# pawanjay176/kzg_rust

Measured on AMD Instinct MI355X. Metric: blobs/sec on verify_blob_kzg_proof_batch (mainnet 4096, batch=64), higher is better.
Workload: dtype u32 limbs (29-bit) / 64-bit accumulate, u8 bytes

## Files before the change

### __graft_entry__.py

```python
import os
import subprocess
import sys

ROOT = os.path.dirname(os.path.abspath(__file__))
if ROOT not in sys.path:
    sys.path.insert(0, ROOT)


def build() -> None:
    env = dict(os.environ)
    subprocess.run(["make", "-C", os.path.join(ROOT, "kzg_rust_amd", "csrc"), "-j5"], check=True, env=env)
    subprocess.run(["make", "-C", os.path.join(ROOT, "oracle")], check=True, env=env)
    native = os.path.join(ROOT, "tests", "native")
    subprocess.run(["g++", "-O2", "-shared", "-fPIC", "-o", os.path.join(native, "libhd_probe.so"), os.path.join(native, "hd_probe.cpp")],
                   check=True, env=env)
    subprocess.run(["g++", "-O2", "-shared", "-fPIC", "-o", os.path.join(native, "liblazy_chain_probe.so"), os.path.join(native, "lazy_chain_probe.cpp")],
                   check=True, env=env)
    subprocess.run(["g++", "-std=c++17", "-O2", "-o", os.path.join(native, "cpp_vector_runner"), os.path.join(native, "cpp_vector_runner.cpp"),
                    "-L" + os.path.join(ROOT, "kzg_rust_amd"), "-lkzg355", "-Wl,-rpath," + os.path.join(ROOT, "kzg_rust_amd")], check=True, env=env)
    subprocess.run(["g++", "-std=c++17", "-O2", "-o", os.path.join(native, "cpp_cell_runner"), os.path.join(native, "cpp_cell_runner.cpp"),
                    "-L" + os.path.join(ROOT, "kzg_rust_amd"), "-lkzg355", "-Wl,-rpath," + os.path.join(ROOT, "kzg_rust_amd")], check=True, env=env)
    subprocess.run(["g++", "-std=c++17", "-O2", "-o", os.path.join(native, "cpp_cell_compute_runner"), os.path.join(native, "cpp_cell_compute_runner.cpp"),
                    "-L" + os.path.join(ROOT, "kzg_rust_amd"), "-lkzg355", "-Wl,-rpath," + os.path.join(ROOT, "kzg_rust_amd")], check=True, env=env)
    subprocess.run(["g++", "-std=c++17", "-O2", "-o", os.path.join(native, "cpp_cell_recover_runner"), os.path.join(native, "cpp_cell_recover_runner.cpp"),
                    "-L" + os.path.join(ROOT, "kzg_rust_amd"), "-lkzg355", "-Wl,-rpath," + os.path.join(ROOT, "kzg_rust_amd")], check=True, env=env)
    quad_src, quad_bin = os.path.join(native, "quad_ops_test.hip"), os.path.join(native, "quad_ops_test")
    quad_deps = [quad_src] + [os.path.join(ROOT, "kzg_rust_amd", "csrc", f) for f in ("g1_quad.h", "g1.h", "field.h", "modinv.h", "consts_gen.h")]
    if not os.path.exists(quad_bin) or any(os.path.getmtime(d) > os.path.getmtime(quad_bin) for d in quad_deps):
        subprocess.run(["/opt/rocm/bin/hipcc", "-O3", "-std=c++17", "--offload-arch=gfx950", "-Wno-unused-result", "-o", quad_bin, quad_src], check=True, env=env)
    probe_src, probe_so = os.path.join(native, "gpu_probe.hip"), os.path.join(native, "libgpu_probe.so")
    probe_deps = [probe_src] + [os.path.join(ROOT, "kzg_rust_amd", "csrc", f) for f in ("field.h", "modinv.h", "eval_core.h", "consts_gen.h")]
    if not os.path.exists(probe_so) or any(os.path.getmtime(d) > os.path.getmtime(probe_so) for d in probe_deps):
        subprocess.run(["/opt/rocm/bin/hipcc", "-O3", "-std=c++17", "--offload-arch=gfx950", "-Wno-unused-result", "-shared", "-fPIC", "-o", probe_so, probe_src],
                       check=True, env=env)
    group_src, group_so = os.path.join(native, "gpu_group_probe.hip"), os.path.join(native, "libgpu_group_probe.so")
    group_deps = [group_src] + [os.path.join(ROOT, "kzg_rust_amd", "csrc", f) for f in
                                ("field.h", "modinv.h", "tower.h", "g1.h", "pairing.h", "pairing_coop.h", "pairing_lanes.h", "consts_gen.h")]
    if not os.path.exists(group_so) or any(os.path.getmtime(d) > os.path.getmtime(group_so) for d in group_deps):
        subprocess.run(["/opt/rocm/bin/hipcc", "-O3", "-std=c++17", "--offload-arch=gfx950", "-Wno-unused-result", "-shared", "-fPIC", "-o", group_so, group_src],
                       check=True, env=env)
    import kzg_rust_amd
    from kzg_rust_amd import _lib
    lib = _lib.load()
    for name in _lib.EXPORTED_SYMBOLS:
        getattr(lib, name)
    print("build ok:", lib.kzg355_version().decode())


def smoke() -> None:
    import torch
    assert torch.cuda.is_available(), "smoke() needs a GPU"
    import kzg_rust_amd as kz
    from oracle.oracle import Oracle
    sys.path.insert(0, os.path.join(ROOT, "tests"))
    from synth import random_blob
    golden = os.path.join(ROOT, "tests", "golden")
    g1 = open(os.path.join(golden, "trusted_setup_g1.bin"), "rb").read()
    g2 = open(os.path.join(golden, "trusted_setup_g2.bin"), "rb").read()
    s = kz.Kzg.load_trusted_setup([g1[48 * i:48 * i + 48] for i in range(4096)], [g2[96 * i:96 * i + 96] for i in range(65)])
    o = Oracle()
    os_ = o.load_trusted_setup(g1, g2)
    blobs = [random_blob(1000 + i) for i in range(3)]
    cs = [kz.Kzg.blob_to_kzg_commitment(kz.Blob(b), s) for b in blobs]
    assert [c.to_bytes() for c in cs] == [o.blob_to_kzg_commitment(b, os_) for b in blobs], "commitment mismatch vs oracle"
    ps = [kz.Kzg.compute_blob_kzg_proof(kz.Blob(b), c, s) for b, c in zip(blobs, cs)]
    assert [p.to_bytes() for p in ps] == [o.compute_blob_kzg_proof(b, c.to_bytes(), os_) for b, c in zip(blobs, cs)], "proof mismatch vs oracle"
    ok = kz.Kzg.verify_blob_kzg_proof_batch([kz.Blob(b) for b in blobs], cs, ps, s)
    assert ok is True and o.verify_blob_kzg_proof_batch(blobs, [c.to_bytes() for c in cs], [p.to_bytes() for p in ps], os_) is True
    bad = [ps[1], ps[0], ps[2]]
    assert kz.Kzg.verify_blob_kzg_proof_batch([kz.Blob(b) for b in blobs], cs, bad, s) is False
    s.free()
    o.free_trusted_setup(os_)
    print("smoke ok: commit/prove bit-exact vs oracle, verify batch true/false as expected")


if __name__ == "__main__":
    build()
    if len(sys.argv) > 1 and sys.argv[1] == "smoke":
        smoke()
```

### kzg_rust_amd/csrc/g1.h

```cpp
#pragma once
#include "field.h"

#if defined(KZG_MID_INLINE)
#define KZG_G1_MID KZG_HD
#else
#define KZG_G1_MID KZG_HD_NOINLINE
#endif

namespace kzg {

struct G1Affine { Fp x, y; };
struct G1Jac { Fp x, y, z; };

KZG_HD G1Jac g1_inf() { G1Jac r; r.x = fp_zero(); r.y = fp_zero(); r.z = fp_zero(); return r; }
KZG_HD G1Affine g1a_inf() { G1Affine r; r.x = fp_zero(); r.y = fp_zero(); return r; }
KZG_HD bool g1_is_inf(const G1Jac &a) { return fp_is_zero(a.z); }
KZG_HD bool g1a_is_inf(const G1Affine &a) { return fp_is_zero(a.x) && fp_is_zero(a.y); }
KZG_HD void g1_neg(G1Jac &r, const G1Jac &a) { r.x = a.x; r.z = a.z; fp_neg(r.y, a.y); }
KZG_HD void g1a_neg(G1Affine &r, const G1Affine &a) { r.x = a.x; fp_neg(r.y, a.y); }
KZG_HD void g1_from_affine(G1Jac &r, const G1Affine &a) {
    bool inf = g1a_is_inf(a);
    r.x = a.x; r.y = a.y;
    Fp one = fp_one(), zero = fp_zero();
    fp_select(r.z, inf, one, zero);
// ... 34 lines not shown
    fp_sub(H, U2, a.x);
    fp_sub(R, S2, a.y);
    if (fp_is_zero(H)) {
        if (fp_is_zero(R)) { G1Jac d = a; g1_dbl(r, d); } else { r = g1_inf(); }
        return;
    }
    fp_sqr(HH, H); fp_mul(HHH, H, HH); fp_mul(V, a.x, HH);
    Fp X3, Y3;
    fp_sqr(X3, R); fp_sub(X3, X3, HHH); fp_sub(X3, X3, V); fp_sub(X3, X3, V);
    fp_sub(t, V, X3); fp_mul(Y3, R, t);
    fp_mul(t, a.y, HHH); fp_sub(Y3, Y3, t);
    fp_mul(r.z, a.z, H);
    r.x = X3; r.y = Y3;
}

KZG_G1_MID void g1_add(G1Jac &r, const G1Jac &a, const G1Jac &b) {
    if (g1_is_inf(a)) { r = b; return; }
    if (g1_is_inf(b)) { r = a; return; }
    Fp Z1Z1, Z2Z2, U1, U2, S1, S2, H, R, HH, HHH, V, t;
    fp_sqr(Z1Z1, a.z); fp_sqr(Z2Z2, b.z);
    fp_mul(U1, a.x, Z2Z2); fp_mul(U2, b.x, Z1Z1);
    fp_mul(S1, a.y, b.z); fp_mul(S1, S1, Z2Z2);
    fp_mul(S2, b.y, a.z); fp_mul(S2, S2, Z1Z1);
    fp_sub(H, U2, U1);
    fp_sub(R, S2, S1);
    if (fp_is_zero(H)) {
        if (fp_is_zero(R)) { G1Jac d = a; g1_dbl(r, d); } else { r = g1_inf(); }
        return;
    }
    fp_sqr(HH, H); fp_mul(HHH, H, HH); fp_mul(V, U1, HH);
    Fp X3, Y3, Z3;
    fp_sqr(X3, R); fp_sub(X3, X3, HHH); fp_sub(X3, X3, V); fp_sub(X3, X3, V);
    fp_sub(t, V, X3); fp_mul(Y3, R, t);
    fp_mul(t, S1, HHH); fp_sub(Y3, Y3, t);
    fp_mul(Z3, a.z, b.z); fp_mul(Z3, Z3, H);
    r.x = X3; r.y = Y3; r.z = Z3;
}

struct G1X { Fp x, y, zz, zzz; };
KZG_HD G1X g1x_inf() { G1X r; r.x = fp_zero(); r.y = fp_zero(); r.zz = fp_zero(); r.zzz = fp_zero(); return r; }
KZG_HD bool g1x_is_inf(const G1X &a) { return fp_is_zero(a.zz); }
KZG_G1_MID void g1x_add_mixed(G1X &r, const G1X &a, const G1Affine &b) {
    if (g1a_is_inf(b)) { r = a; return; }
    if (g1x_is_inf(a)) { r.x = b.x; r.y = b.y; r.zz = fp_one(); r.zzz = fp_one(); return; }
    Fp U2, S2, P, R, PP, PPP, Q, t;
    fp_mul(U2, b.x, a.zz);
    fp_mul(S2, b.y, a.zzz);
    fp_sub(P, U2, a.x);
    fp_sub(R, S2, a.y);
    if (fp_is_zero(P)) {
        if (!fp_is_zero(R)) { r = g1x_inf(); return; }
        Fp U, V, W, S, M;
        fp_dbl(U, b.y); fp_sqr(V, U); fp_mul(W, U, V); fp_mul(S, b.x, V);
        fp_sqr(M, b.x); fp_dbl(t, M); fp_add(M, M, t);
        Fp X3, Y3;
        fp_sqr(X3, M); fp_sub(X3, X3, S); fp_sub(X3, X3, S);
        fp_sub(t, S, X3); fp_mul(Y3, M, t); fp_mul(t, W, b.y); fp_sub(Y3, Y3, t);
        r.x = X3; r.y = Y3; r.zz = V; r.zzz = W;
        return;
    }
    fp_sqr(PP, P); fp_mul(PPP, P, PP); fp_mul(Q, a.x, PP);
    Fp X3, Y3;
    fp_sqr(X3, R); fp_sub(X3, X3, PPP); fp_sub(X3, X3, Q); fp_sub(X3, X3, Q);
    fp_sub(t, Q, X3); fp_mul(Y3, R, t);
    fp_mul(t, a.y, PPP); fp_sub(Y3, Y3, t);
    fp_mul(r.zz, a.zz, PP);
    fp_mul(r.zzz, a.zzz, PPP);
    r.x = X3; r.y = Y3;
}
KZG_HD void g1_lazy_x3(Fp &X3, Fp &t, const Fp &RR, const Fp &PPP, const Fp &Q) {
    const uint32_t m2[NFP] = FP_MOD2_INIT, m8[NFP] = FP_MOD8_INIT;
    Fp u;
    fp_sub_lz(t, RR, PPP, m2);
    fp_sub_lz(u, t, Q, m2);
    fp_sub_lz(X3, u, Q, m2);
    fp_sub_lz(t, Q, X3, m8);
}
KZG_HD void g1_lazy_y3(Fp &Y3, const Fp &R, const Fp &t, const Fp &S1, const Fp &PPP) {
    const uint32_t m2[NFP] = FP_MOD2_INIT;
    Fp u;
    { const Fp z = fp_zero(); fp_sub_lz(u, z, S1, m2); }
    fp_mul2_lz(Y3, R, t, u, PPP);
}
KZG_G1_MID void g1x_add_mixed_lazy(G1X &acc, bool &started, const G1Affine &b) {
    const uint32_t m2[NFP] = FP_MOD2_INIT, m4[NFP] = FP_MOD4_INIT, m8[NFP] = FP_MOD8_INIT;
    if (!started) {
        if (g1a_is_inf(b)) return;
        acc.x = b.x; acc.y = b.y; acc.zz = fp_one(); acc.zzz = fp_one(); started = true;
        return;
    }
    Fp U2, S2, P, R;
    fp_mul_lz(U2, b.x, acc.zz);
    fp_mul_lz(S2, b.y, acc.zzz);
    fp_sub_lz(P, U2, acc.x, m8);
    fp_sub_lz(R, S2, acc.y, m4);
    if (fp_maybe_zero_lz(P) || g1a_is_inf(b)) {
        G1X c; fp_canon16(c.x, acc.x); fp_canon16(c.y, acc.y); fp_canon16(c.zz, acc.zz); fp_canon16(c.zzz, acc.zzz);
        g1x_add_mixed(c, c, b);
        acc = c;
        started = !g1x_is_inf(c);
        return;
    }
    Fp PP, PPP, Q, t, u;
    fp_sqr_lz(PP, P); fp_mul_lz(PPP, P, PP); fp_mul_lz(Q, acc.x, PP);
    Fp X3, Y3;
    fp_sqr_lz(X3, R);
    fp_sub_lz(t, X3, PPP, m2);
    fp_sub_lz(u, t, Q, m2);
    fp_sub_lz(X3, u, Q, m2);
    fp_sub_lz(t, Q, X3, m8);
#if defined(KZG_G1_ADD_MUL2)
    { const Fp z = fp_zero(); fp_sub_lz(u, z, acc.y, m4); }
    fp_mul2_lz(Y3, R, t, u, PPP);
#else
    fp_mul_lz(Y3, R, t);
    fp_mul_lz(t, acc.y, PPP);
    fp_sub_lz(Y3, Y3, t, m2);
#endif
    fp_mul_lz(acc.zz, acc.zz, PP);
    fp_mul_lz(acc.zzz, acc.zzz, PPP);
    acc.x = X3; acc.y = Y3;
}
KZG_G1_MID void g1x_from_lazy(G1X &r, const G1X &acc, bool started) {
    if (!started) { r = g1x_inf(); return; }
    fp_canon16(r.x, acc.x); fp_canon16(r.y, acc.y); fp_canon16(r.zz, acc.zz); fp_canon16(r.zzz, acc.zzz);
}

KZG_G1_MID void g1x_to_jac(G1Jac &r, const G1X &a) {
    if (g1x_is_inf(a)) { r = g1_inf(); return; }
    fp_mul(r.x, a.x, a.zz);
    fp_mul(r.y, a.y, a.zzz);
    r.z = a.zz;
}

KZG_G1_MID void g1x_add_lazy2(G1X &r, const G1X &a, const G1X &b) {
    const uint32_t m2[NFP] = FP_MOD2_INIT;
    Fp U1, U2, S1, S2, ZZ12, ZZZ12, P, R;
    fp_mul_lz(U1, a.x, b.zz); fp_mul_lz(U2, b.x, a.zz);
    fp_mul_lz(S1, a.y, b.zzz); fp_mul_lz(S2, b.y, a.zzz);
    fp_mul_lz(ZZ12, a.zz, b.zz); fp_mul_lz(ZZZ12, a.zzz, b.zzz);
    fp_sub_lz(P, U2, U1, m2);
    fp_sub_lz(R, S2, S1, m2);
    if (fp_maybe_zero_lz(P) || fp_maybe_zero_lz(a.zz) || fp_maybe_zero_lz(b.zz)) {
        G1X ca, cb; g1x_from_lazy(ca, a, true); g1x_from_lazy(cb, b, true);
        G1Jac ja, jb, jr; g1x_to_jac(ja, ca); g1x_to_jac(jb, cb);
        g1_add(jr, ja, jb);
        if (g1_is_inf(jr)) { r = g1x_inf(); return; }
        r.x = jr.x; r.y = jr.y; fp_sqr(r.zz, jr.z); fp_mul(r.zzz, r.zz, jr.z);
        return;
    }
    Fp PP, PPP, Q, t, X3, Y3;
    fp_sqr_lz(PP, P); fp_mul_lz(PPP, P, PP); fp_mul_lz(Q, U1, PP);
    fp_sqr_lz(X3, R);
    g1_lazy_x3(X3, t, X3, PPP, Q);
    g1_lazy_y3(Y3, R, t, S1, PPP);
    fp_mul_lz(r.zz, ZZ12, PP);
    fp_mul_lz(r.zzz, ZZZ12, PPP);
    r.x = X3; r.y = Y3;
}


struct PairPt { Fp ax, ay, az; };
KZG_G1_MID void pairpt_from_jac(PairPt &r, const G1Jac &a, bool negate) {
    if (g1_is_inf(a)) { r.ax = fp_zero(); r.ay = fp_zero(); r.az = fp_zero(); return; }
    Fp z2;
    fp_mul(r.ax, a.x, a.z);
    fp_sqr(z2, a.z); fp_mul(r.az, z2, a.z);
    r.ay = a.y;
    if (negate) fp_neg(r.ay, r.ay);
}
KZG_HD void pairpt_from_affine(PairPt &r, const G1Affine &a) {
    if (g1a_is_inf(a)) { r.ax = fp_zero(); r.ay = fp_zero(); r.az = fp_zero(); return; }
    r.ax = a.x; r.ay = a.y; r.az = fp_one();
}
KZG_G1_MID void g1_to_affine(G1Affine &r, const G1Jac &a) {
    if (g1_is_inf(a)) { r = g1a_inf(); return; }
    Fp zi, zi2, zi3;
    fp_inv(zi, a.z); fp_sqr(zi2, zi); fp_mul(zi3, zi2, zi);
    fp_mul(r.x, a.x, zi2); fp_mul(r.y, a.y, zi3);
}
KZG_G1_MID void pairpt_to_affine(G1Affine &r, const PairPt &a) {
    if (fp_is_zero(a.az)) { r = g1a_inf(); return; }
    Fp zi; fp_inv(zi, a.az);
    fp_mul(r.x, a.ax, zi); fp_mul(r.y, a.ay, zi);
}

KZG_HD void g1_mul_words(G1Jac &r, const G1Affine &p, const uint32_t *k, int nwords) {
    G1Jac acc = g1_inf();
    for (int w = nwords - 1; w >= 0; w--) {
        uint32_t x = k[w];
        for (int b = 0; b < 32; b++) {
            g1_dbl(acc, acc);
            if (x >> 31) g1_add_mixed(acc, acc, p);
            x <<= 1;
        }
    }
    r = acc;
}

KZG_G1_MID void g1_dbl_lazy(G1Jac &r, const G1Jac &p) {
    const uint32_t m2[NFP] = FP_MOD2_INIT, m4[NFP] = FP_MOD4_INIT, m8[NFP] = FP_MOD8_INIT;
// ... 239 lines not shown
```

### kzg_rust_amd/csrc/k_g1.hip

```cpp
#if !defined(KZG_G1_TU_NOINLINE)
#define KZG_MID_INLINE 1
#else
#define KZG_FP_MUL_NOINLINE 1
#endif
#include "kernels.h"
#include "g1_quad.h"

namespace kzg {

template <bool SUBGROUP>
__device__ __forceinline__ void decode_point_to_slot(const uint8_t *commitments, const uint8_t *proofs, int n_total, int n_per_group, G1Affine *pts, int *err,
        int stride) {
    const int j = blockIdx.x * blockDim.x + threadIdx.x;
    if (j >= 2 * n_total) return;
    const bool is_proof = j >= n_total;
    if (is_proof && !proofs) return;
    const int i = is_proof ? j - n_total : j;
    const uint8_t *src = (is_proof ? proofs : commitments) + (size_t)stride * i;
    uint8_t b[48];
    for (int k = 0; k < 48; k++) b[k] = src[k];
    G1Affine p;
    int rc = g1_decompress(p, b);
    if (SUBGROUP && rc == 0 && !g1a_is_inf(p) && !g1_in_subgroup(p)) rc = 3;
    const int g = i / n_per_group, k = i % n_per_group;
// ... 127 lines not shown
    if (c >= 2) return;
    G1Jac acc = g1_inf();
    for (int wv = 0; wv < wpg; wv++) { G1Jac v = partials[((size_t)g * wpg + wv) * 2 + c]; g1_add(acc, acc, v); }
    PairPt a; pairpt_from_jac(a, acc, c == 0);
    pair_pts[2 * (size_t)g + c] = a;
}

__global__ void __launch_bounds__(64) k_lincomb_single(const G1Affine *pts, const uint32_t *scal_b, const uint32_t *scal_c, int groups, PairPt *pair_pts,
                                                        uint32_t *wtabs) {
    const int lane = threadIdx.x, q = lane & 3;
    const int g_raw = blockIdx.x * 16 + (lane >> 2);
    const bool live = g_raw < groups;
    const int g = live ? g_raw : groups - 1;
    uint32_t *wtab = wtabs + (size_t)blockIdx.x * (W4_ENTRIES * 3 * NFP * 64);
    const G1Affine *gp = pts + 2 * (size_t)g;
    G1Affine p; uint32_t k[8];
    if (q < 2) { p = gp[1]; for (int w = 0; w < 8; w++) k[w] = scal_b[8 * (size_t)g + w]; }
    else { p = g1a_neg_gen(); for (int w = 0; w < 8; w++) k[w] = scal_c[8 * (size_t)g + w]; }
    uint32_t ka[4], kb[4];
    glv_split_fast(ka, kb, k);
    if (q & 1) { G1Affine t; g1a_neg_phi(t, p); p = t; }
    G1Jac m;
    g1_mul128_w4(m, p, (q & 1) ? kb : ka, wtab, lane);
    G1Jac c; g1_from_affine(c, gp[0]);
#pragma unroll 1
    for (int it = 0; it < 3; it++) {
        G1Jac o = g1_shfl_xor(m, it == 0 ? 1 : 2);
        if (it == 2) o = c;
        g1_add(m, m, o);
    }
    if (!live) return;
    if (q == 0) { PairPt a; pairpt_from_jac(a, m, false); pair_pts[2 * (size_t)g + 1] = a; }
    if (q == 1) {
        G1Jac pj; g1_from_affine(pj, gp[1]);
        PairPt a; pairpt_from_jac(a, pj, true); pair_pts[2 * (size_t)g] = a;
    }
}

constexpr int LC_BITS = 5;
constexpr int LC_BUCKETS = 1 << (LC_BITS - 1);
constexpr int LC_WINDOWS = 26;
constexpr int LC_DIG_STRIDE = 28;
__host__ __device__ inline int lc_items(int n) { return 2 * (3 * n + 1); }

__global__ void __launch_bounds__(64) k_lc_prep(const G1Affine *pts, const uint32_t *scal_a, const uint32_t *scal_b, const uint32_t *scal_c, int n,
                                                 G1Affine *items, int8_t *digits) {
    const int nt = 3 * n + 1, bpg = (nt + 63) / 64;
    const int g = blockIdx.x / bpg, t = (blockIdx.x % bpg) * 64 + threadIdx.x;
    if (t >= nt) return;
    const G1Affine *gp = pts + (size_t)g * 2 * n;
    G1Affine p; uint32_t k[8];
    if (t < n) { p = gp[n + t]; for (int q = 0; q < 8; q++) k[q] = scal_a[8 * ((size_t)g * n + t) + q]; }
    else if (t < 2 * n) { p = gp[n + (t - n)]; for (int q = 0; q < 8; q++) k[q] = scal_b[8 * ((size_t)g * n + (t - n)) + q]; }
    else if (t < 3 * n) { p = gp[t - 2 * n]; for (int q = 0; q < 8; q++) k[q] = scal_a[8 * ((size_t)g * n + (t - 2 * n)) + q]; }
    else { p = g1a_neg_gen(); for (int q = 0; q < 8; q++) k[q] = scal_c[8 * (size_t)g + q]; }
    uint32_t half[2][4];
    glv_split(half[0], half[1], k);
    G1Affine q2; g1a_neg_phi(q2, p);
    const size_t base = (size_t)g * lc_items(n) + 2 * (size_t)t;
    items[base] = p; items[base + 1] = q2;
    const uint32_t bias[4] = {0x21084210u, 0x08421084u, 0x42108421u, 0x10842108u};
    for (int h = 0; h < 2; h++) {
        uint32_t e[6]; uint64_t c = 0;
        for (int i = 0; i < 4; i++) { c += (uint64_t)half[h][i] + bias[i]; e[i] = (uint32_t)c; c >>= 32; }
        e[4] = (uint32_t)c; e[5] = 0;
        int8_t *d = digits + (base + h) * LC_DIG_STRIDE;
        for (int w = 0; w < LC_WINDOWS; w++) {
            const int bit = LC_BITS * w;
            const uint64_t two = (uint64_t)e[bit >> 5] | ((uint64_t)e[(bit >> 5) + 1] << 32);
            const int chunk = (int)((two >> (bit & 31)) & 31u);
            d[w] = (int8_t)(w < LC_WINDOWS - 1 ? chunk - 16 : chunk);
        }
    }
}

constexpr int LC_TASKS = 13;
constexpr int LC_LDS_LIST = 400;
constexpr int LC_MAX_LISTS = 8;
__host__ __device__ inline int lc_list_stride(int n) { return 2 * (2 * n + 1) + 2; }
__host__ __device__ inline int lc_wave_n1(int wid) { return wid < 2 ? 7 : 6; }
__host__ __device__ inline int lc_wave_c1w0(int wid) { return wid < 2 ? 7 * wid : 14 + 6 * (wid - 2); }
__host__ __device__ inline int lc_wave_c0w0(int wid) { return wid < 2 ? 6 * wid : 12 + 7 * (wid - 2); }
union LcSlot { G1X raw; G1Jac jac; };
__global__ void __launch_bounds__(256) k_lc_buckets(const G1Affine *items, const int8_t *digits, int n, LcSlot *S, uint16_t *glists, int keep_raw) {
    __shared__ uint16_t lists_all[4][LC_TASKS * LC_LDS_LIST];
    __shared__ int cnt_all[4][LC_TASKS][LC_BUCKETS + 1], cursor_all[4][LC_TASKS][LC_BUCKETS + 1];
    __shared__ uint8_t order_all[4][LC_BUCKETS * LC_TASKS];
    __shared__ uint8_t seq_all[4][64][LC_MAX_LISTS];
    const int g = blockIdx.x, wid = threadIdx.x >> 6, lane = threadIdx.x & 63;
    const int n1 = lc_wave_n1(wid), c1w0 = lc_wave_c1w0(wid), c0w0 = lc_wave_c0w0(wid);
    constexpr int ntasks = LC_TASKS, nlists = LC_BUCKETS * LC_TASKS;
    int (*cnt)[LC_BUCKETS + 1] = cnt_all[wid], (*cursor)[LC_BUCKETS + 1] = cursor_all[wid];
    uint8_t *order = order_all[wid];
    uint8_t (*seq)[LC_MAX_LISTS] = seq_all[wid];
    const int ni = lc_items(n);
    const G1Affine *it = items + (size_t)g * ni;
    const int8_t *dg = digits + (size_t)g * ni * LC_DIG_STRIDE;
    const bool in_lds = 40 * n + 14 <= LC_TASKS * LC_LDS_LIST;
    uint16_t *lists = in_lds ? lists_all[wid] : glists + ((size_t)blockIdx.x * 4 + wid) * LC_TASKS * lc_list_stride(n);
    LcSlot *out = S + (size_t)g * 2 * LC_WINDOWS * LC_BUCKETS;
    auto task_window = [&](int tk) { return tk < n1 ? c1w0 + tk : c0w0 + (tk - n1); };
    auto slot_of = [&](int L) { const int tk = L / LC_BUCKETS; return ((tk < n1 ? 1 : 0) * LC_WINDOWS + task_window(tk)) * LC_BUCKETS + (L % LC_BUCKETS); };
    auto len_of = [&](int L) { return cnt[L / LC_BUCKETS][(L % LC_BUCKETS) + 1]; };
    for (int q = lane; q < (LC_BUCKETS + 1) * LC_TASKS; q += 64) cnt[q / (LC_BUCKETS + 1)][q % (LC_BUCKETS + 1)] = 0;
    __syncthreads();
#pragma unroll 1
    for (int tk = 0; tk < ntasks; tk++) {
        const int w = task_window(tk), lo = tk < n1 ? 2 * n : 0, hi = tk < n1 ? ni : 2 * n;
        for (int j = lo + lane; j < hi; j += 64) { const int d = dg[(size_t)j * LC_DIG_STRIDE + w]; if (d) atomicAdd(&cnt[tk][d < 0 ? -d : d], 1); }
    }
    __syncthreads();
#pragma unroll 1
    for (int L = lane; L < nlists; L += 64) {
        const int len = len_of(L);
        int rank = 0;
        for (int M = 0; M < nlists; M++) { const int lm = len_of(M); rank += (lm > len) || (lm == len && M < L); }
        order[rank] = (uint8_t)L;
        if (len == 0) { if (keep_raw) out[slot_of(L)].raw = g1x_inf(); else out[slot_of(L)].jac = g1_inf(); }
    }
    __syncthreads();
    int total = 0, nmine = 0;
    {
        const int L = order[lane], len = len_of(L);
        if (len > 0) { seq[lane][0] = (uint8_t)L; total = len; nmine = 1; }
    }
#pragma unroll 1
    for (int r = 64; r < nlists; r++) {
        const int L = order[r], len = len_of(L);
        if (len == 0) break;
        int key = nmine >= LC_MAX_LISTS ? 0x7fffffff : (total << 6) | lane;
#pragma unroll
        for (int off = 32; off > 0; off >>= 1) { const int v = __shfl_xor(key, off); key = v < key ? v : key; }
        if (lane == (key & 63) && nmine < LC_MAX_LISTS) { seq[lane][nmine++] = (uint8_t)L; total += len; }
    }
    int lane_start = total;
#pragma unroll
    for (int off = 1; off < 64; off <<= 1) { const int v = __shfl_up(lane_start, off); if (lane >= off) lane_start += v; }
    lane_start -= total;
    {
        int run = lane_start;
#pragma unroll 1
        for (int k = 0; k < nmine; k++) { const int L = seq[lane][k]; cursor[L / LC_BUCKETS][(L % LC_BUCKETS) + 1] = run; run += len_of(L); }
    }
    __syncthreads();
#pragma unroll 1
    for (int tk = 0; tk < ntasks; tk++) {
        const int w = task_window(tk), lo = tk < n1 ? 2 * n : 0, hi = tk < n1 ? ni : 2 * n;
        for (int j = lo + lane; j < hi; j += 64) {
            const int d = dg[(size_t)j * LC_DIG_STRIDE + w];
            if (d) { const int pos = atomicAdd(&cursor[tk][d < 0 ? -d : d], 1); lists[pos] = (uint16_t)(j | (d < 0 ? 0x8000 : 0)); }
        }
    }
    __threadfence_block();
    __syncthreads();
    int tmax = total, kmax = nmine;
#pragma unroll
    for (int off = 32; off > 0; off >>= 1) { const int v = __shfl_xor(tmax, off), u = __shfl_xor(kmax, off); tmax = v > tmax ? v : tmax;
            kmax = u > kmax ? u : kmax; }
    {
        G1X accx = g1x_inf(); bool started = false;
        const uint16_t *lst = lists + lane_start;
        auto entry = [&](int q) -> uint32_t { return q < total ? (in_lds ? (uint32_t)lst[q] : (uint32_t)__builtin_nontemporal_load(lst + q)) : 0u; };
        uint32_t v0 = entry(0), v1 = entry(1);
        G1Affine pn = it[v0 & 0x7fff];
        int k = 0, cur = nmine ? (int)seq[lane][0] : 0, end = nmine ? len_of(cur) : 0;
#pragma unroll 1
        for (int q = 0; q < tmax; q++) {
            if (q < total) {
                G1Affine p = pn;
                const uint32_t v = v0;
                v0 = v1; v1 = entry(q + 2);
                pn = it[v0 & 0x7fff];
                if (v & 0x8000) fp_neg(p.y, p.y);
                g1x_add_mixed_lazy(accx, started, p);
                if (q + 1 == end) {
                    if (!started) accx = g1x_inf();
                    out[slot_of(cur)].raw = accx;
                    started = false;
                    k++;
                    if (k < nmine) { cur = seq[lane][k]; end += len_of(cur); }
                }
            }
        }
    }
    if (keep_raw) return;
#pragma unroll 1
    for (int k = 0; k < kmax; k++) {
        if (k >= nmine) continue;
        LcSlot *sl = out + slot_of(seq[lane][k]);
        G1X raw = sl->raw, cx;
        g1x_from_lazy(cx, raw, true);
        G1Jac acc; g1x_to_jac(acc, cx);
        sl->jac = acc;
    }
}

__global__ void __launch_bounds__(256) k_lc_horner(const LcSlot *S, int groups, PairPt *pair_pts) {
    const int id = blockIdx.x * blockDim.x + threadIdx.x;
    const int lane = threadIdx.x & 63;
    const bool live = id < 2 * LC_BUCKETS * groups;
    const int gc = live ? id / LC_BUCKETS : 0, bi = id % LC_BUCKETS;
    const LcSlot *s = S + (size_t)gc * LC_WINDOWS * LC_BUCKETS;
    G1Jac acc = live ? s[(size_t)(LC_WINDOWS - 1) * LC_BUCKETS + bi].jac : g1_inf();
#pragma unroll 1
    for (int k = LC_BITS * (LC_WINDOWS - 1) - 1; k >= 0; k--) {
        g1_dbl_lazy(acc, acc);
        if (k % LC_BITS == 0) { G1Jac v = live ? s[(size_t)(k / LC_BITS) * LC_BUCKETS + bi].jac : g1_inf(); g1_add_lazy(acc, acc, v); }
    }
    g1_canon_lazy(acc, acc);
    G1Jac r = acc;
#pragma unroll 1
    for (int off = 1; off < LC_BUCKETS; off <<= 1) {
        G1Jac o = g1_shfl_down16(r, off), t;
        g1_add(t, r, o);
        if ((lane % LC_BUCKETS) + off < LC_BUCKETS) r = t;
    }
#pragma unroll 1
    for (int off = 1; off < LC_BUCKETS; off <<= 1) { G1Jac o = g1_shfl_xor(r, off); g1_add(r, r, o); }
    if (!live || bi != 0) return;
    PairPt a; pairpt_from_jac(a, r, (gc & 1) == 0);
    pair_pts[gc] = a;
}

__global__ void __launch_bounds__(256, 2) k_lc_wsum(const LcSlot *S, int groups, G1Jac *W) {
    __shared__ uint32_t tot[4 * NFP][256];
    const int id = blockIdx.x * blockDim.x + threadIdx.x, tid = threadIdx.x;
    if (id >= 2 * LC_WINDOWS * groups) return;
    const LcSlot *s = S + (size_t)id * LC_BUCKETS;
    int start = -1;
#pragma unroll 1
    for (int b = LC_BUCKETS - 1; b >= 0 && start < 0; b--) {
        const Fp zz = s[b].raw.zz;
        uint32_t o = 0;
#pragma unroll
        for (int i = 0; i < NFP; i++) o |= zz.l[i];
        if (o) start = b;
    }
    if (start < 0) { W[id] = g1_inf(); return; }
    G1X acc = s[start].raw;
#pragma unroll
    for (int i = 0; i < NFP; i++) { tot[i][tid] = acc.x.l[i]; tot[NFP + i][tid] = acc.y.l[i]; tot[2 * NFP + i][tid] = acc.zz.l[i];
            tot[3 * NFP + i][tid] = acc.zzz.l[i]; }
#pragma unroll 1
    for (int b = LC_BUCKETS - 2; b >= 0; b--) {
        if (b >= start) continue;
        g1x_add_lazy2(acc, acc, s[b].raw);
        asm volatile("" ::: "memory");
        G1X sum;
#pragma unroll
        for (int i = 0; i < NFP; i++) { sum.x.l[i] = tot[i][tid]; sum.y.l[i] = tot[NFP + i][tid]; sum.zz.l[i] = tot[2 * NFP + i][tid];
                sum.zzz.l[i] = tot[3 * NFP + i][tid]; }
        g1x_add_lazy2(sum, sum, acc);
#pragma unroll
        for (int i = 0; i < NFP; i++) { tot[i][tid] = sum.x.l[i]; tot[NFP + i][tid] = sum.y.l[i]; tot[2 * NFP + i][tid] = sum.zz.l[i];
                tot[3 * NFP + i][tid] = sum.zzz.l[i]; }
        asm volatile("" ::: "memory");
    }
// ... 183 lines not shown
    uint8_t b[48]; g1_compress_affine(b, p);
    for (int k = 0; k < 48; k++) o[32 + 48 * which + k] = b[k];
    if (which == 0) {
        const uint32_t *r = scal_a + 8 * ((size_t)g * n + (n > 1 ? 1 : 0));
        for (int k = 0; k < 8; k++) { const uint32_t v = r[7 - k]; o[4 * k] = (uint8_t)(v >> 24); o[4 * k + 1] = (uint8_t)(v >> 16);
                o[4 * k + 2] = (uint8_t)(v >> 8); o[4 * k + 3] = (uint8_t)v; }
    }
}
void launch_dump_intermediates(const uint32_t *d_scal_a, const PairPt *d_pair_pts, int n_per_group, int groups, uint8_t *d_out, hipStream_t st) {
    if (groups <= 0) return;
    hipLaunchKernelGGL(k_dump_intermediates, dim3((2 * groups + 63) / 64), dim3(64), 0, st, d_scal_a, d_pair_pts, n_per_group, groups, d_out);
}
void launch_decompress_points(const uint8_t *d_commitments, const uint8_t *d_proofs, int n_total, int n_per_group, G1Affine *d_pts, int *d_err, hipStream_t st,
        int stride) {
    if (n_total <= 0) return;
    hipLaunchKernelGGL(k_decompress_points, dim3((2 * n_total + 63) / 64), dim3(64), 0, st, d_commitments, d_proofs, n_total, n_per_group, d_pts, d_err,
            stride);
}
void launch_subgroup_points(const G1Affine *d_pts, int n_total, int n_per_group, int *d_err, hipStream_t st, int commitments_only) {
    if (n_total <= 0) return;
    if (2 * n_total <= 1024) {
        hipLaunchKernelGGL(k_subgroup_points_quad, dim3((8 * n_total + 255) / 256), dim3(256), 0, st, d_pts, 2 * n_total, n_per_group, d_err, commitments_only);
        return;
    }
    hipLaunchKernelGGL(k_subgroup_points, dim3((2 * n_total + 63) / 64), dim3(64), 0, st, d_pts, 2 * n_total, n_per_group, d_err, commitments_only);
}
void launch_subgroup_ladder_from_x(const uint8_t *d_commitments, int stride, int n, G1Jac *d_T, hipStream_t st) {
    if (n <= 0) return;
    hipLaunchKernelGGL(k_subgroup_ladder_from_x_quad, dim3((4 * n + 255) / 256), dim3(256), 0, st, d_commitments, stride, n, d_T);
}
void launch_subgroup_finish(const G1Affine *d_pts, const G1Jac *d_T, int n, int *d_err, hipStream_t st) {
    if (n <= 0) return;
    hipLaunchKernelGGL(k_subgroup_finish, dim3((n + 63) / 64), dim3(64), 0, st, d_pts, d_T, n, d_err);
}
void launch_points_from_records(const uint8_t *d_records, int n_total, int n_per_group, G1Affine *d_pts, int *d_err, hipStream_t st) {
    if (n_total <= 0) return;
    hipLaunchKernelGGL(k_points_from_records, dim3((2 * n_total + 63) / 64), dim3(64), 0, st, d_records, n_total, n_per_group, d_pts, d_err);
}
void launch_lincomb(const G1Affine *d_pts, const uint32_t *d_scal_a, const uint32_t *d_scal_b, const uint32_t *d_scal_c, int n_per_group,
                    int groups, G1Jac *d_partials, PairPt *d_pair_pts, hipStream_t st) {
    if (groups <= 0) return;
    const int wpg = lincomb_waves_per_group(n_per_group);
    uint32_t *d_wtabs = reinterpret_cast<uint32_t *>(d_partials + 2 * (size_t)wpg * groups);
    hipLaunchKernelGGL(k_lincomb_terms, dim3(groups * wpg), dim3(64), 0, st, d_pts, d_scal_a, d_scal_b, d_scal_c, n_per_group, d_partials, d_wtabs);
    hipLaunchKernelGGL(k_lincomb_finish, dim3(groups), dim3(64), 0, st, d_partials, n_per_group, d_pair_pts);
}
size_t lincomb_single_bytes(int groups) { return sizeof(uint32_t) * W4_ENTRIES * 3 * NFP * 64 * (size_t)((groups + 15) / 16); }
void launch_lincomb_single(const G1Affine *d_pts, const uint32_t *d_scal_b, const uint32_t *d_scal_c, int groups, void *d_scratch, PairPt *d_pair_pts,
                           hipStream_t st) {
    if (groups <= 0) return;
    hipLaunchKernelGGL(k_lincomb_single, dim3((groups + 15) / 16), dim3(64), 0, st, d_pts, d_scal_b, d_scal_c, groups, d_pair_pts,
            reinterpret_cast<uint32_t *>(d_scratch));
}
static size_t lc_glists_entries(int n_per_group, int groups) {
    if (40 * (size_t)n_per_group + 14 <= (size_t)LC_TASKS * LC_LDS_LIST) return 0;
    return (((size_t)groups * 4 * LC_TASKS * lc_list_stride(n_per_group)) + 7) & ~(size_t)7;
}
struct LcScratch {
    G1Affine *items; LcSlot *S; int8_t *digits; uint16_t *glists; G1Jac *W;
    size_t bytes;
    LcScratch(void *d_scratch, int n_per_group, int groups) {
        const size_t ni = (size_t)lc_items(n_per_group) * groups;
        uintptr_t at = reinterpret_cast<uintptr_t>(d_scratch);
        auto take = [&](size_t nbytes) { const uintptr_t r = at; at += nbytes; return r; };
        items = reinterpret_cast<G1Affine *>(take(ni * sizeof(G1Affine)));
        S = reinterpret_cast<LcSlot *>(take((size_t)2 * LC_WINDOWS * LC_BUCKETS * groups * sizeof(LcSlot)));
        const size_t dig = ni * LC_DIG_STRIDE, dig_padded = (dig + 255) & ~(size_t)255;
        digits = reinterpret_cast<int8_t *>(take(dig_padded));
        glists = reinterpret_cast<uint16_t *>(take(lc_glists_entries(n_per_group, groups) * sizeof(uint16_t)));
        W = reinterpret_cast<G1Jac *>(take((size_t)2 * LC_WINDOWS * groups * sizeof(G1Jac)));
        bytes = (size_t)(at - reinterpret_cast<uintptr_t>(d_scratch)) - (dig_padded - dig) + 512;
    }
};
static void launch_lc_prep(const G1Affine *d_pts, const uint32_t *d_scal_a, const uint32_t *d_scal_b, const uint32_t *d_scal_c, int n_per_group, int groups,
        const LcScratch &sc, hipStream_t st) {
    const int nt = 3 * n_per_group + 1;
    hipLaunchKernelGGL(k_lc_prep, dim3(groups * ((nt + 63) / 64)), dim3(64), 0, st, d_pts, d_scal_a, d_scal_b, d_scal_c, n_per_group, sc.items, sc.digits);
}
void launch_lincomb_buckets(const G1Affine *d_pts, const uint32_t *d_scal_a, const uint32_t *d_scal_b, const uint32_t *d_scal_c, int n_per_group,
                            int groups, void *d_scratch, PairPt *d_pair_pts, hipStream_t st, int stage, int chain_from) {
    if (groups <= 0) return;
    const LcScratch sc(d_scratch, n_per_group, groups);
    if (stage == 0 || stage == 1) launch_lc_prep(d_pts, d_scal_a, d_scal_b, d_scal_c, n_per_group, groups, sc, st);
    if (stage == 0 || stage == 2) hipLaunchKernelGGL(k_lc_buckets, dim3(groups), dim3(256), 0, st, sc.items, sc.digits, n_per_group, sc.S, sc.glists,
            groups >= chain_from ? 1 : 0);
    if (stage == 0 || stage == 3) {
        if (groups >= chain_from) {
            hipLaunchKernelGGL(k_lc_wsum, dim3((2 * LC_WINDOWS * groups + 255) / 256), dim3(256), 0, st, sc.S, groups, sc.W);
            hipLaunchKernelGGL(k_lc_hchain_quad, dim3((8 * groups + 255) / 256), dim3(256), 0, st, sc.W, groups, d_pair_pts);
        } else hipLaunchKernelGGL(k_lc_horner, dim3((2 * LC_BUCKETS * groups + 255) / 256), dim3(256), 0, st, sc.S, groups, d_pair_pts);
    }
}
size_t lincomb_buckets_scratch_bytes(int n_per_group, int groups) {
    return LcScratch(nullptr, n_per_group, groups).bytes;
}
bool lincomb_preshift_fits(int n_per_group, int groups) { return n_per_group >= 1 && n_per_group <= PS_MAX_N && groups >= 1 && groups < 64; }
size_t lincomb_preshift_bytes(int n_per_group, int groups) { return sizeof(G1Jac) * (size_t)ps_points(n_per_group) * LC_WINDOWS * groups; }
static void launch_ps_shift(const G1Affine *d_pts, const uint8_t *d_commitments, const uint8_t *d_proofs, int stride, int n_per_group, int groups,
        G1Jac *d_shifts, hipStream_t st) {
    if (groups <= 0) return;
    const int total = ps_points(n_per_group) * groups;
    hipLaunchKernelGGL(k_ps_shift, dim3((4 * total + PS_SHIFT_THREADS - 1) / PS_SHIFT_THREADS), dim3(PS_SHIFT_THREADS), 0, st, d_pts, d_commitments, d_proofs,
            stride, n_per_group, groups, d_shifts);
}
void launch_lincomb_preshift(const G1Affine *d_pts, int n_per_group, int groups, G1Jac *d_shifts, hipStream_t st) {
    launch_ps_shift(d_pts, nullptr, nullptr, 0, n_per_group, groups, d_shifts, st);
}
void launch_lincomb_preshift_bytes(const uint8_t *d_commitments, const uint8_t *d_proofs, int stride, int n_per_group, int groups, G1Jac *d_shifts,
        hipStream_t st) {
    launch_ps_shift(nullptr, d_commitments, d_proofs, stride, n_per_group, groups, d_shifts, st);
}
void launch_lincomb_preshifted(const G1Affine *d_pts, const G1Jac *d_shifts, const uint32_t *d_scal_a, const uint32_t *d_scal_b, const uint32_t *d_scal_c,
        int n_per_group,
                               int groups, void *d_scratch, PairPt *d_pair_pts, hipStream_t st, int stage) {
    if (groups <= 0) return;
    const LcScratch sc(d_scratch, n_per_group, groups);
    if (stage == 0 || stage == 1) launch_lc_prep(d_pts, d_scal_a, d_scal_b, d_scal_c, n_per_group, groups, sc, st);
    if (stage == 1) return;
    hipLaunchKernelGGL(k_ps_buckets, dim3(2 * groups * LC_BUCKETS), dim3(PS_THREADS), 0, st, d_shifts, d_pts, sc.digits, n_per_group, sc.S);
    hipLaunchKernelGGL(k_ps_weights, dim3(2 * groups), dim3(64), 0, st, sc.S, groups, d_pair_pts);
}
size_t lincomb_partials_bytes(int n_per_group, int groups) {
    const size_t waves = (size_t)lincomb_waves_per_group(n_per_group) * groups;
    return sizeof(G1Jac) * 2 * waves + sizeof(uint32_t) * W4_ENTRIES * 3 * NFP * 64 * waves;
}

}
```

Before: 4.575 million.

## Stage bucket-accumulation points in LDS and use fused mul2 in mixed add

When a group's point table is small enough (2n+1 ≤ 169 rows), k_lc_buckets first copies the points into shared memory as packed rows that hold both the x-halves and the shared y. The bucket-add loop then reads each point from LDS instead of gathering it from global memory. The LDS path also switches the mixed addition to the fused mul2 Y3 formula through a template parameter. This adds roughly 28KB of LDS per block and a fill loop, which may lower occupancy.

```diff
diff --git a/__graft_entry__.py b/__graft_entry__.py
--- a/__graft_entry__.py
+++ b/__graft_entry__.py
@@ -16,6 +16,8 @@
                    check=True, env=env)
     subprocess.run(["g++", "-O2", "-shared", "-fPIC", "-o", os.path.join(native, "liblazy_chain_probe.so"), os.path.join(native, "lazy_chain_probe.cpp")],
                    check=True, env=env)
+    subprocess.run(["g++", "-O2", "-shared", "-fPIC", "-o", os.path.join(native, "libadd_mixed_forms_probe.so"),
+                    os.path.join(native, "add_mixed_forms_probe.cpp")], check=True, env=env)
     subprocess.run(["g++", "-std=c++17", "-O2", "-o", os.path.join(native, "cpp_vector_runner"), os.path.join(native, "cpp_vector_runner.cpp"),
                     "-L" + os.path.join(ROOT, "kzg_rust_amd"), "-lkzg355", "-Wl,-rpath," + os.path.join(ROOT, "kzg_rust_amd")], check=True, env=env)
     subprocess.run(["g++", "-std=c++17", "-O2", "-o", os.path.join(native, "cpp_cell_runner"), os.path.join(native, "cpp_cell_runner.cpp"),
diff --git a/kzg_rust_amd/csrc/g1.h b/kzg_rust_amd/csrc/g1.h
--- a/kzg_rust_amd/csrc/g1.h
+++ b/kzg_rust_amd/csrc/g1.h
@@ -140,7 +140,12 @@
     { const Fp z = fp_zero(); fp_sub_lz(u, z, S1, m2); }
     fp_mul2_lz(Y3, R, t, u, PPP);
 }
-KZG_G1_MID void g1x_add_mixed_lazy(G1X &acc, bool &started, const G1Affine &b) {
+#if defined(KZG_G1_ADD_MUL2)
+constexpr bool G1_ADD_MUL2_DEFAULT = true;
+#else
+constexpr bool G1_ADD_MUL2_DEFAULT = false;
+#endif
+template <bool MUL2 = G1_ADD_MUL2_DEFAULT> KZG_G1_MID void g1x_add_mixed_lazy(G1X &acc, bool &started, const G1Affine &b) {
     const uint32_t m2[NFP] = FP_MOD2_INIT, m4[NFP] = FP_MOD4_INIT, m8[NFP] = FP_MOD8_INIT;
     if (!started) {
         if (g1a_is_inf(b)) return;
@@ -167,14 +172,14 @@
     fp_sub_lz(u, t, Q, m2);
     fp_sub_lz(X3, u, Q, m2);
     fp_sub_lz(t, Q, X3, m8);
-#if defined(KZG_G1_ADD_MUL2)
-    { const Fp z = fp_zero(); fp_sub_lz(u, z, acc.y, m4); }
-    fp_mul2_lz(Y3, R, t, u, PPP);
-#else
-    fp_mul_lz(Y3, R, t);
-    fp_mul_lz(t, acc.y, PPP);
-    fp_sub_lz(Y3, Y3, t, m2);
-#endif
+    if constexpr (MUL2) {
+        { const Fp z = fp_zero(); fp_sub_lz(u, z, acc.y, m4); }
+        fp_mul2_lz(Y3, R, t, u, PPP);
+    } else {
+        fp_mul_lz(Y3, R, t);
+        fp_mul_lz(t, acc.y, PPP);
+        fp_sub_lz(Y3, Y3, t, m2);
+    }
     fp_mul_lz(acc.zz, acc.zz, PP);
     fp_mul_lz(acc.zzz, acc.zzz, PPP);
     acc.x = X3; acc.y = Y3;
diff --git a/kzg_rust_amd/csrc/k_g1.hip b/kzg_rust_amd/csrc/k_g1.hip
--- a/kzg_rust_amd/csrc/k_g1.hip
+++ b/kzg_rust_amd/csrc/k_g1.hip
@@ -233,6 +233,10 @@
 __host__ __device__ inline int lc_wave_c1w0(int wid) { return wid < 2 ? 7 * wid : 14 + 6 * (wid - 2); }
 __host__ __device__ inline int lc_wave_c0w0(int wid) { return wid < 2 ? 6 * wid : 12 + 7 * (wid - 2); }
 union LcSlot { G1X raw; G1Jac jac; };
+constexpr int LC_ROW_WORDS = 3 * NFP / 2;
+constexpr int LC_LDS_POINTS = 169;
+static_assert(NFP % 2 == 0 && sizeof(G1Affine) == 2 * NFP * sizeof(uint32_t), "a point is 14 + 14 dwords, copied as 64-bit words");
+template <bool LDS_PTS>
 __global__ void __launch_bounds__(256) k_lc_buckets(const G1Affine *items, const int8_t *digits, int n, LcSlot *S, uint16_t *glists, int keep_raw) {
     __shared__ uint16_t lists_all[4][LC_TASKS * LC_LDS_LIST];
     __shared__ int cnt_all[4][LC_TASKS][LC_BUCKETS + 1], cursor_all[4][LC_TASKS][LC_BUCKETS + 1];
@@ -253,6 +257,17 @@
     auto task_window = [&](int tk) { return tk < n1 ? c1w0 + tk : c0w0 + (tk - n1); };
     auto slot_of = [&](int L) { const int tk = L / LC_BUCKETS; return ((tk < n1 ? 1 : 0) * LC_WINDOWS + task_window(tk)) * LC_BUCKETS + (L % LC_BUCKETS); };
     auto len_of = [&](int L) { return cnt[L / LC_BUCKETS][(L % LC_BUCKETS) + 1]; };
+    const uint2 *ptab = nullptr;
+    if constexpr (LDS_PTS) {
+        __shared__ uint2 ptab_all[LC_LDS_POINTS * LC_ROW_WORDS];
+        const uint2 *src = reinterpret_cast<const uint2 *>(it);
+        const int words = (2 * n + 1) * LC_ROW_WORDS;
+        for (int q = threadIdx.x; q < words; q += 256) {
+            const int row = q / LC_ROW_WORDS, c = q % LC_ROW_WORDS, j = 2 * (n + row);
+            ptab_all[q] = src[c < NFP / 2 ? j * NFP + c : c < NFP ? (j + 1) * NFP + (c - NFP / 2) : j * NFP + (c - NFP / 2)];
+        }
+        ptab = ptab_all;
+    }
     for (int q = lane; q < (LC_BUCKETS + 1) * LC_TASKS; q += 64) cnt[q / (LC_BUCKETS + 1)][q % (LC_BUCKETS + 1)] = 0;
     __syncthreads();
 #pragma unroll 1
@@ -313,17 +328,30 @@
         const uint16_t *lst = lists + lane_start;
         auto entry = [&](int q) -> uint32_t { return q < total ? (in_lds ? (uint32_t)lst[q] : (uint32_t)__builtin_nontemporal_load(lst + q)) : 0u; };
         uint32_t v0 = entry(0), v1 = entry(1);
-        G1Affine pn = it[v0 & 0x7fff];
+        G1Affine pn;
+        if constexpr (!LDS_PTS) pn = it[v0 & 0x7fff];
         int k = 0, cur = nmine ? (int)seq[lane][0] : 0, end = nmine ? len_of(cur) : 0;
 #pragma unroll 1
         for (int q = 0; q < tmax; q++) {
             if (q < total) {
-                G1Affine p = pn;
+                G1Affine p;
                 const uint32_t v = v0;
                 v0 = v1; v1 = entry(q + 2);
-                pn = it[v0 & 0x7fff];
-                if (v & 0x8000) fp_neg(p.y, p.y);
-                g1x_add_mixed_lazy(accx, started, p);
+                if constexpr (LDS_PTS) {
+                    const int t = (int)(v & 0x7fff) >> 1, h = (int)(v & 1);
+                    const uint2 *row = ptab + (t < n ? t : t - n) * LC_ROW_WORDS;
+#pragma unroll
+                    for (int i = 0; i < NFP / 2; i++) {
+                        const uint2 a = row[h * (NFP / 2) + i], b = row[NFP + i];
+                        p.x.l[2 * i] = a.x; p.x.l[2 * i + 1] = a.y; p.y.l[2 * i] = b.x; p.y.l[2 * i + 1] = b.y;
+                    }
+                    if (((v >> 15) ^ v) & 1) fp_neg(p.y, p.y);
+                } else {
+                    p = pn;
+                    pn = it[v0 & 0x7fff];
+                    if (v & 0x8000) fp_neg(p.y, p.y);
+                }
+                g1x_add_mixed_lazy<LDS_PTS>(accx, started, p);
                 if (q + 1 == end) {
                     if (!started) accx = g1x_inf();
                     out[slot_of(cur)].raw = accx;
@@ -673,8 +701,10 @@
     if (groups <= 0) return;
     const LcScratch sc(d_scratch, n_per_group, groups);
     if (stage == 0 || stage == 1) launch_lc_prep(d_pts, d_scal_a, d_scal_b, d_scal_c, n_per_group, groups, sc, st);
-    if (stage == 0 || stage == 2) hipLaunchKernelGGL(k_lc_buckets, dim3(groups), dim3(256), 0, st, sc.items, sc.digits, n_per_group, sc.S, sc.glists,
-            groups >= chain_from ? 1 : 0);
+    if (stage == 0 || stage == 2) {
+        auto *buckets = 2 * n_per_group + 1 <= LC_LDS_POINTS ? k_lc_buckets<true> : k_lc_buckets<false>;
+        hipLaunchKernelGGL(buckets, dim3(groups), dim3(256), 0, st, sc.items, sc.digits, n_per_group, sc.S, sc.glists, groups >= chain_from ? 1 : 0);
+    }
     if (stage == 0 || stage == 3) {
         if (groups >= chain_from) {
             hipLaunchKernelGGL(k_lc_wsum, dim3((2 * LC_WINDOWS * groups + 255) / 256), dim3(256), 0, st, sc.S, groups, sc.W);
```

Result: no change. 4.609 million, median of 6 (+0.7%).
